# StefanHeng/Symbolic-Music-Generation

Hardware: AMD Instinct MI355X
Metric: train tokens/sec (TransfoXL seq2048 bf16), whole job (higher is better)
Workload: dtype bf16; 1 GPU; TransfoXL 12L/768d H12 dh64 F3072 T=2048 M=2048 V=1190 cutoffs=[] (SURVEY C3, mode R: fresh zero mems); per_gpu_batch=64, global_batch=64, seq_len=2048, mem_len=2048, parallelism=dp1

## Files before the change

### include/musicxl.h

```cpp
#ifndef MUSICXL_H
#define MUSICXL_H

#ifdef __cplusplus
extern "C" {
#endif

#define MXL_ABI_VERSION 2

int mxl_abi_version(void);
const char* mxl_error_string(int code);

#define MXL_GEMM_OUT_F32        0x01
#define MXL_GEMM_OUT_F32_ATOMIC 0x02
#define MXL_GEMM_BIAS           0x04
#define MXL_GEMM_RELU           0x08
#define MXL_GEMM_DROPOUT        0x10
#define MXL_GEMM_RELU_BWD       0x20
#define MXL_GEMM_ADD_AUX        0x40
int mxl_set_reserved_cus(int k);
int mxl_gemm_last_nt_kernel(void);

#define MXL_GEMM_SAVE_RELU_MASK 0x100
#define MXL_GEMM_RELU_BWD_BITS  0x200
size_t mxl_gemm_relu_mask_bytes(int M, int N);
// ... 46 lines not shown
int mxl_relattn_fwd_phantom(const void* q, const void* k, const void* v, const void* rd, const float* r_w_bias,
                            const float* r_r_bias, void* out, float* lse, void* oph, float* mph, int B, int T, int H,
                            int dh, int M, int Kc, long long q_bs, int q_rs, long long kv_bs, int kv_rs, int rd_rs,
                            long long o_bs, int o_rs, float scale, void* stream);
int mxl_relattn_bwd_sparse_dg_oph(const void* q, const void* k, const void* v, const void* rd, const float* r_w_bias,
                                  const float* r_r_bias, const void* out, const void* dout, const float* lse,
                                  float* delta, void* dq, void* dk, void* dv, void* dg, float* d_r_w_bias,
                                  const void* oph, const float* mph, int B, int T, int H, int dh, int M, int Kc,
                                  long long q_bs, int q_rs, long long kv_bs, int kv_rs, int rd_rs, long long o_bs, int o_rs,
                                  long long dq_bs, int dq_rs, long long dkv_bs, int dkv_rs, float scale, void* stream);
int mxl_relattn_drd_recompute(const void* dg, const void* qr, float* d_rd, int B, int T, int H, int dh, int M, long long qr_bs,
                              int qr_rs, int drd_ld, const void* rd, int rd_rs, float* d_r_r_bias, float* d_r_w_bias_fix,
                              const float* lse, const float* delta, float scale, int Kc, void* stream);

size_t mxl_relattn_bwd_fused_ws_bytes(int B, int T, int H, int dh, int M);
int mxl_relattn_bwd_fused(const void* q, const void* k, const void* v, const void* rd, const float* r_w_bias,
                          const float* r_r_bias, const void* out, const void* dout, const float* lse, float* delta,
                          void* dq, void* dk, void* dv, float* d_rd, int drd_ld, float* d_r_w_bias, float* d_r_r_bias,
                          const void* oph, const float* mph, void* ws, int B, int T, int H, int dh, int M, int Kc,
                          long long q_bs, int q_rs, long long kv_bs, int kv_rs, int rd_rs, long long o_bs, int o_rs,
                          long long dq_bs, int dq_rs, long long dkv_bs, int dkv_rs, float scale, int defer_finish, void* stream);
int mxl_relattn_dq_finish(const void* ws, const void* oph, const float* mph, const float* lse, const float* delta, void* dq,
                          float* d_r_r_bias, int B, int T, int H, int dh, int M, int Kc, long long o_bs, int o_rs, long long dq_bs,
                          int dq_rs, float scale, void* stream);
int mxl_relattn_fwd_phantom2(const void* q, const void* k, const void* v, const void* rd, const float* r_w_bias,
                             const float* r_r_bias, void* out, float* lse, void* oph, float* mph, int oph_all, void* ph_ws, int B,
                             int T, int H, int dh, int M, int Kc, long long q_bs, int q_rs, long long kv_bs, int kv_rs, int rd_rs,
                             long long o_bs, int o_rs, float scale, void* stream);
size_t mxl_relattn_drd_phantom_ws_bytes(int B, int T, int H);
int mxl_relattn_drd_phantom_prep(const void* q, long long q_bs, int q_rs, const float* r_r_bias, const float* lse, void* ws, int B, int T,
                                 int H, int dh, float scale, void* stream);
int mxl_relattn_drd_phantom(const void* ws, const float* delta, float* d_rd, int B, int T, int H, int dh, int M, int drd_ld,
                            const void* rd, int rd_rs, int Kc, void* stream);

int mxl_sinusoid_table(void* out, int M, int d, int clamp_len, float drop_p, unsigned long long seed, unsigned site,
                       void* stream);
int mxl_embed_fwd(const void* ids, const void* E, void* out, int N, int d, int V, float scale, float drop_p,
                  unsigned long long seed, unsigned site, void* stream);
int mxl_embed_bwd(const void* ids, const void* dout, const void* dout2, float* dE, int N, int d, int V, float scale,
                  float drop_p, unsigned long long seed, unsigned site, void* stream);
int mxl_dropout_bf16(const void* x, void* y, long long n, float drop_p, unsigned long long seed, unsigned site,
                     void* stream);
int mxl_ln_residual_fwd(const void* x, const void* res, const float* gamma, const float* beta, void* y, void* z,
                        float* mean, float* rstd, int N, int d, float eps, float drop_p, unsigned long long seed,
                        unsigned site, void* stream);
int mxl_ln_residual_bwd(const void* dy, const void* dy2, const void* z, const float* mean, const float* rstd,
                        const float* gamma, void* dres, void* dx, float* dgamma, float* dbeta, int N, int d,
                        float drop_p, unsigned long long seed, unsigned site, void* stream);
int mxl_ln_residual_bwd_colsum(const void* dy, const void* dy2, const void* z, const float* mean, const float* rstd,
                               const float* gamma, void* dres, void* dx, float* dgamma, float* dbeta, float* dxsum, int N,
                               int d, float drop_p, unsigned long long seed, unsigned site, void* stream);
int mxl_ln_residual_bwd_add(const void* dy, const void* dy2, const void* z, const float* mean, const float* rstd,
                            const float* gamma, const void* dadd, void* dres, float* dgamma, float* dbeta, int N, int d,
                            void* stream);
int mxl_ln_residual_bwd_add_drop(const void* dy, const void* dy2, const void* z, const float* mean, const float* rstd,
                                 const float* gamma, const void* dadd, void* dres, void* dx, float* dxsum, float* dgamma,
                                 float* dbeta, int N, int d, float drop_p, unsigned long long seed, unsigned site, void* stream);
int mxl_add_rowbias_bf16(const void* x, long long x_bs, int x_rs, const float* bias, void* out, int B, int T, int n,
                         void* stream);
int mxl_colsum_bf16(const void* X, float* out, int M, int N, int ld, void* stream);
int mxl_dropout_colsum_bf16(const void* X, void* Y, float* out, int M, int N, float drop_p, unsigned long long seed,
                            unsigned site, void* stream);
int mxl_center_columns_bf16(const void* X, void* Y, int M, int N, void* stream);
int mxl_mem_update(const void* mem, const void* hid, void* out, int B, int M, int T, int d, void* stream);

int mxl_label_guard(void* labels_row0, int T, long long eos, void* stream);
// ... 200 lines not shown
```

### symbolic_music_generation_amd/csrc/common.h

```cpp
#pragma once
#include <hip/hip_runtime.h>
#include <stdint.h>

#define MXL_OK 0
#define MXL_EINVAL (-1)
#define MXL_EUNSUPPORTED (-2)

#define MXL_CHECK_ARG(cond) do { if (!(cond)) return MXL_EINVAL; } while (0)
#define MXL_LAUNCH_CHECK() do { hipError_t e_ = hipGetLastError(); if (e_ != hipSuccess) return (int)e_; } while (0)

typedef uint16_t bf16_t;

using bf16x8 = __attribute__((ext_vector_type(8))) short;
using bf16x4 = __attribute__((ext_vector_type(4))) short;
using f32x4 = __attribute__((ext_vector_type(4))) float;
using f32x16 = __attribute__((ext_vector_type(16))) float;
using u32x4 = __attribute__((ext_vector_type(4))) uint32_t;
using u32x2 = __attribute__((ext_vector_type(2))) uint32_t;

__device__ __forceinline__ float bf2f(bf16_t x) { return __uint_as_float(((uint32_t)x) << 16); }

__device__ __forceinline__ bf16_t f2bf(float f) {
    __bf16 b = (__bf16)f;
    return __builtin_bit_cast(bf16_t, b);
}
__device__ __forceinline__ uint32_t pack2bf(float lo, float hi) {
    typedef __bf16 bf2_t __attribute__((ext_vector_type(2)));
    typedef float f2_t __attribute__((ext_vector_type(2)));
    f2_t v = {lo, hi};
    bf2_t r = __builtin_convertvector(v, bf2_t);
    return __builtin_bit_cast(uint32_t, r);
}

__device__ __forceinline__ void xcd_block(int& bx, int& by, int& bz) {
    const int gx = gridDim.x, gy = gridDim.y, groups = gridDim.y * gridDim.z;
#ifndef MXL_NO_XCD_REMAP
    const int L = blockIdx.x + gx * (blockIdx.y + gy * blockIdx.z);
    const int xcd = L & 7, idx = L >> 3;
    int grp;
    if ((groups & 7) == 0) {
        grp = (idx / gx) * 8 + xcd;
        bx = idx % gx;
    } else {
        const int n = gx * groups, q = n >> 3, r = n & 7;
        const int id = (xcd < r ? xcd * (q + 1) : r * (q + 1) + (xcd - r) * q) + idx;
        grp = id / gx;
        bx = id - grp * gx;
    }
    by = grp % gy; bz = grp / gy;
#else
    bx = blockIdx.x; by = blockIdx.y; bz = blockIdx.z;
#endif
}

__device__ __forceinline__ int lane_id() { return threadIdx.x & 63; }

__device__ __forceinline__ float wave_sum(float v) {
#pragma unroll
    for (int o = 32; o > 0; o >>= 1) v += __shfl_xor(v, o, 64);
    return v;
}
__device__ __forceinline__ float wave_max(float v) {
#pragma unroll
    for (int o = 32; o > 0; o >>= 1) v = fmaxf(v, __shfl_xor(v, o, 64));
    return v;
}

__device__ __forceinline__ uint32_t mxl_hash32(uint32_t x) {
    x ^= x >> 16; x *= 0x7feb352dU; x ^= x >> 15; x *= 0x846ca68bU; x ^= x >> 16;
    return x;
}
__device__ __forceinline__ bool dropout_keep(uint64_t seed, uint32_t site, uint64_t idx, uint32_t thresh) {
    const uint32_t mix = mxl_hash32((uint32_t)seed ^ (site * 0x9E3779B9U)) + (uint32_t)(seed >> 32);
    const uint32_t h = mxl_hash32(((uint32_t)idx * 0x9E3779B1U) ^ ((uint32_t)(idx >> 32) * 0x85EBCA77U) ^ mix);
    return h >= thresh;
}
__device__ __forceinline__ bool dropout_keep32(uint64_t seed, uint32_t site, uint32_t idx, uint32_t thresh) {
    const uint32_t mix = mxl_hash32((uint32_t)seed ^ (site * 0x9E3779B9U)) + (uint32_t)(seed >> 32);
    return mxl_hash32((idx * 0x9E3779B1U) ^ mix) >= thresh;
}
static inline uint32_t dropout_thresh(float p) {
// ... 6 lines not shown
```

### symbolic_music_generation_amd/csrc/relattn_bwd_fused.hip

```cpp
#include <cstdlib>
#include <type_traits>
#include "common.h"
#include "musicxl_internal.h"

namespace {

typedef __attribute__((ext_vector_type(8))) __bf16 mfma_bf16x8;
typedef __attribute__((address_space(3))) bf16x4 lds_bf16x4;
typedef _Float16 f16x4 __attribute__((ext_vector_type(4)));
typedef float f32x4v __attribute__((ext_vector_type(4)));

#ifndef FUSED_PF
#define FUSED_PF 3
#endif
#ifndef FUSED_VF_RELOAD
#define FUSED_VF_RELOAD 0
#endif
#ifndef FUSED_PARK
#define FUSED_PARK 0
#endif
#ifndef FUSED_SB
#define FUSED_SB 1
#endif
#define UNIT_FENCE() do { if (FUSED_SB) __builtin_amdgcn_sched_barrier(0); } while (0)
// ... 33 lines not shown
#ifdef MXL_STAMP
__device__ unsigned long long g_fused_stamps[16];
#define STAMP_DECL unsigned long long st_last, st_acc[16] = {0ull, 0ull, 0ull, 0ull, 0ull, 0ull, 0ull, 0ull, 0ull, 0ull, 0ull, 0ull, 0ull, 0ull, 0ull, 0ull}; \
    { __builtin_amdgcn_sched_barrier(0); asm volatile("s_memtime %0\n\ts_waitcnt lgkmcnt(0)" : "=s"(st_last) :: "memory"); __builtin_amdgcn_sched_barrier(0); }
#define STAMP(i) { unsigned long long t_; __builtin_amdgcn_sched_barrier(0); asm volatile("s_memtime %0\n\ts_waitcnt lgkmcnt(0)" : "=s"(t_) :: "memory"); \
    __builtin_amdgcn_sched_barrier(0); st_acc[i] += t_ - st_last; st_last = t_; }
#define STAMP_FLUSH if ((threadIdx.x & 63) == 0) { for (int i_ = 0; i_ < 16; i_++) atomicAdd(&g_fused_stamps[i_], st_acc[i_]); }
#else
#define STAMP_DECL
#define STAMP(i)
#define STAMP_FLUSH
#endif

#ifndef MXL_SLAB_BF16
#define MXL_SLAB_BF16 1
#endif
#if MXL_SLAB_BF16
typedef bf16_t slab_t;
#else
typedef float slab_t;
#endif

struct FusedP {
    const bf16_t *q, *k, *v, *rd, *dout;
    const float *rwb, *rrb, *lse, *delta;
    bf16_t *dk, *dv;
    slab_t* slab;
    float* drd;
    float *d_rwb, *d_rrb;
    int B, T, H, M, Kc;
    long long q_bs, kv_bs, o_bs, dkv_bs, slab_stride;
    int q_rs, kv_rs, rd_rs, o_rs, dkv_rs, drd_ld;
    float scale, scale_log2e;
};

__device__ __forceinline__ int qswz(int row) { return (((row >> 1) & 1) << 2) | (((row >> 2) & 1) << 1) | ((row >> 3) & 1); }
__device__ __forceinline__ int qoff(int row, int ch) { return row * ROWB + ((ch ^ qswz(row)) << 4); }
__device__ __forceinline__ int qeoff(int row, int e) { return qoff(row, e >> 3) + ((e & 7) << 1); }
__device__ __forceinline__ int sswz(int row) { return (((row >> 3) & 1) << 2) | (((row >> 1) & 1) << 1) | ((row >> 2) & 1); }
__device__ __forceinline__ int soff(int row, int ch) { return row * ROWB + ((ch ^ sswz(row)) << 4); }

__device__ __forceinline__ void lds_barrier() {
    asm volatile("s_waitcnt lgkmcnt(0)" ::: "memory");
    __builtin_amdgcn_s_barrier();
    asm volatile("" ::: "memory");
}

__device__ __forceinline__ uint32_t lds_addr(const void* p) {
    return (uint32_t)(uintptr_t)(__attribute__((address_space(3))) const char*)(const char*)p;
}

__device__ __forceinline__ void gskew_wait() { asm volatile("s_waitcnt lgkmcnt(0)" ::: "memory"); }
__device__ __forceinline__ void gskew_read16(uint32_t base, uint32_t (&u)[16]) {
    static_assert(GP == 584, "offsets below are pat(j) * (GP + 2)");
    asm volatile(
        "ds_read_u16 %0, %16\n\t"               "ds_read_u16 %1, %16 offset:586\n\t"    "ds_read_u16 %2, %16 offset:1172\n\t"
        "ds_read_u16 %3, %16 offset:1758\n\t"   "ds_read_u16 %4, %16 offset:4688\n\t"   "ds_read_u16 %5, %16 offset:5274\n\t"
        "ds_read_u16 %6, %16 offset:5860\n\t"   "ds_read_u16 %7, %16 offset:6446\n\t"   "ds_read_u16 %8, %16 offset:9376\n\t"
        "ds_read_u16 %9, %16 offset:9962\n\t"   "ds_read_u16 %10, %16 offset:10548\n\t" "ds_read_u16 %11, %16 offset:11134\n\t"
        "ds_read_u16 %12, %16 offset:14064\n\t" "ds_read_u16 %13, %16 offset:14650\n\t" "ds_read_u16 %14, %16 offset:15236\n\t"
        "ds_read_u16 %15, %16 offset:15822"
        : "=&v"(u[0]), "=&v"(u[1]), "=&v"(u[2]), "=&v"(u[3]), "=&v"(u[4]), "=&v"(u[5]), "=&v"(u[6]), "=&v"(u[7]),
          "=&v"(u[8]), "=&v"(u[9]), "=&v"(u[10]), "=&v"(u[11]), "=&v"(u[12]), "=&v"(u[13]), "=&v"(u[14]), "=&v"(u[15])
        : "v"(base)
        : "memory");
}
// ... 41 lines not shown
    const bf16_t* dp = dout + (size_t)b * o_bs + (size_t)i * o_rs;
    const int chunks = H * 8;
    for (int c0 = 0; c0 < chunks; c0 += 64) {
        const int c = c0 + lane;
        float s = 0.f;
        if (c < chunks) {
            const bf16x8 a = *reinterpret_cast<const bf16x8*>(op + c * 8);
            const bf16x8 d = *reinterpret_cast<const bf16x8*>(dp + c * 8);
#pragma unroll
            for (int j = 0; j < 8; j++) s += bf2f((bf16_t)a[j]) * bf2f((bf16_t)d[j]);
        }
        s += __shfl_xor(s, 1, 64); s += __shfl_xor(s, 2, 64); s += __shfl_xor(s, 4, 64);
        if (c < chunks && (lane & 7) == 0) delta[((size_t)b * H + (c >> 3)) * T + i] = s;
    }
}

__global__ __launch_bounds__(512, 1) void relattn_bwd_fused_kernel(FusedP p) {
    constexpr int NT = 512;
    extern __shared__ __attribute__((aligned(16))) char smem[];
    char* sK = smem;
    char* sR = sK + K_BYTES;
    char* sQ = sR + RING_BYTES;
    char* sG = sQ + 2 * QSET;
    char* sX = sG + G_BYTES;
    char* sY = sX + X_BYTES;
    float* sBias = reinterpret_cast<float*>(sY + Y_BYTES);
    float* sPark = sBias + BIAS_BYTES / 4;

    STAMP_DECL
    const int tid = threadIdx.x;
    const int w = __builtin_amdgcn_readfirstlane(tid >> 6);
    const int l = tid & 63, r = l & 31, hh = l >> 5;
    int bx_, h, b;
    xcd_block(bx_, h, b);
    const int T = p.T, M = p.M;
    const int p0 = T - p.Kc;
    const int P0 = p0 + KBLK * bx_;
    const int Pw = P0 + 32 * w;
    const int kloc0 = 32 * w + r;
    const int MB = M >> 5;

    const bf16_t* qbase = p.q + (size_t)b * p.q_bs + (size_t)h * 64;
    const bf16_t* dobase = p.dout + (size_t)b * p.o_bs + (size_t)h * 64;
    const bf16_t* rbase = p.rd + (size_t)h * 64;
    const bf16_t* kbase = p.k + (size_t)b * p.kv_bs + (size_t)h * 64;
    const bf16_t* vbase = p.v + (size_t)b * p.kv_bs + (size_t)h * 64;

    const int gq = l >> 4, q4 = (l & 15) >> 2, pp = l & 3;
    int rowq = qoff(r, hh);
    int rows = r * ROWB + ((hh ^ sswz(r)) << 4);
    int tkb = qeoff(4 * hh + q4, 16 * (gq & 1) + 4 * pp);
    const uint32_t gRb = lds_addr(sG) + 4 * hh * (GP + 2) + (256 - kloc0) * 2;
    const uint32_t yWb = lds_addr(sY) + 4 * hh * (YP + 2) + (256 - kloc0) * 2;
    const int xf = (kloc0 >> 1) & 7;
    int xw = kloc0 * 64 + ((((hh ^ (xf & 1)) | (xf & 6))) << 3);
    int yt0 = (4 * (l >> 4) + ((l & 15) >> 2)) * YP + (16 * (w & 1) + 4 * pp) * 2;
    int qb0 = qeoff(4 * (l >> 4) + ((l & 15) >> 2), 16 * (w >> 1) + 4 * pp);
    const int eq = w >> 1, ih0 = w & 1;
    const int g16 = l >> 4, q16 = (l & 15) >> 2;
    int xa0 = ((8 * g16 + q16) * 64 + ((pp ^ ((4 * g16 + (q16 >> 1)) & 7)) << 3)) ^ (ih0 << 5);
    int xa1 = ((8 * g16 + q16 + 4) * 64 + ((pp ^ ((4 * g16 + 2 + (q16 >> 1)) & 7)) << 3)) ^ (ih0 << 5);
    const int kch = 2 * eq + (pp >> 1);
    const int ksw = ((g16 & 1) << 2) | (((q16 >> 1) & 1) << 1);
    int ka0 = (8 * g16 + q16) * ROWB + ((kch ^ ksw) << 4) + ((pp & 1) << 3);
    int ka1 = (8 * g16 + q16 + 4) * ROWB + ((kch ^ (ksw | 1)) << 4) + ((pp & 1) << 3);
    int yq0 = (16 * ih0 + (l & 15)) * YP + 16 * g16;
    int krow = kloc0 * ROWB + ((hh ^ sswz(kloc0)) << 4);
// ... 649 lines not shown
    MXL_CHECK_ARG(q && k && v && rd && r_w_bias && r_r_bias && out && dout && lse && delta && dq && dk && dv && d_rd && d_r_w_bias &&
                  d_r_r_bias && ws);
    if (dh != 64) return MXL_EUNSUPPORTED;
    MXL_CHECK_ARG(B > 0 && T > 0 && H > 0 && M > 0 && Kc >= T && Kc <= M + T && drd_ld >= H * 64);
    if ((T % 32) != 0 || (M % 32) != 0 || (Kc % 32) != 0) return MXL_EUNSUPPORTED;
    MXL_CHECK_ARG(Kc == M + T || (oph && mph));
    MXL_CHECK_ARG((q_rs % 8) == 0 && (kv_rs % 8) == 0 && (rd_rs % 8) == 0 && (o_rs % 8) == 0 && (dq_rs % 8) == 0 && (dkv_rs % 4) == 0);
    MXL_CHECK_ARG((q_bs % 8) == 0 && (kv_bs % 8) == 0 && (o_bs % 8) == 0 && (dq_bs % 8) == 0 && (dkv_bs % 4) == 0);
    MXL_CHECK_ARG(((uintptr_t)q % 16) == 0 && ((uintptr_t)k % 16) == 0 && ((uintptr_t)v % 16) == 0 && ((uintptr_t)rd % 16) == 0 &&
                  ((uintptr_t)out % 16) == 0 && ((uintptr_t)dout % 16) == 0 && ((uintptr_t)dq % 16) == 0 && ((uintptr_t)ws % 16) == 0 &&
                  (oph == nullptr || ((uintptr_t)oph % 16) == 0));
    hipStream_t s = (hipStream_t)stream;
    static bool attr_set = false;
    if (!attr_set) {
        hipError_t e = hipFuncSetAttribute(reinterpret_cast<const void*>(&relattn_bwd_fused_kernel), hipFuncAttributeMaxDynamicSharedMemorySize, SMEM);
        if (e != hipSuccess) return (int)e;
        attr_set = true;
    }
    const bool delta_ready = (defer_finish & 2) != 0;
    defer_finish &= 1;
    if (!delta_ready) {
        mxl_kt::Scope kt(MXL_KT_RELATTN_DELTA, s);
        hipLaunchKernelGGL(fused_delta_kernel, dim3((B * T + 3) / 4), dim3(256), 0, s, (const bf16_t*)out, (const bf16_t*)dout, delta, B, T,
                           H, o_bs, o_rs);
    }
    FusedP p;
    p.q = (const bf16_t*)q; p.k = (const bf16_t*)k; p.v = (const bf16_t*)v; p.rd = (const bf16_t*)rd; p.dout = (const bf16_t*)dout;
    p.rwb = r_w_bias; p.rrb = r_r_bias; p.lse = lse; p.delta = delta;
    p.dk = (bf16_t*)dk; p.dv = (bf16_t*)dv; p.slab = (slab_t*)ws; p.drd = d_rd; p.d_rwb = d_r_w_bias; p.d_rrb = d_r_r_bias;
    p.B = B; p.T = T; p.H = H; p.M = M; p.Kc = Kc;
    p.q_bs = q_bs; p.kv_bs = kv_bs; p.o_bs = o_bs; p.dkv_bs = dkv_bs; p.slab_stride = (long long)B * T * H * 64;
    p.q_rs = q_rs; p.kv_rs = kv_rs; p.rd_rs = rd_rs; p.o_rs = o_rs; p.dkv_rs = dkv_rs; p.drd_ld = drd_ld;
    p.scale = scale; p.scale_log2e = scale * LOG2E;
    {
        mxl_kt::Scope kt(MXL_KT_RELATTN_FUSED, s);
        hipLaunchKernelGGL(relattn_bwd_fused_kernel, dim3((Kc + KBLK - 1) / KBLK, H, B), dim3(512), SMEM, s, p);
    }
    MXL_LAUNCH_CHECK();
    if (defer_finish) return MXL_OK;
    return mxl_relattn_dq_finish(ws, oph, mph, lse, delta, dq, d_r_r_bias, B, T, H, dh, M, Kc, o_bs, o_rs, dq_bs, dq_rs, scale, stream);
}

extern "C" int mxl_relattn_dq_finish(const void* ws, const void* oph, const float* mph, const float* lse, const float* delta, void* dq,
                                     float* d_r_r_bias, int B, int T, int H, int dh, int M, int Kc, long long o_bs, int o_rs,
                                     long long dq_bs, int dq_rs, float scale, void* stream) {
    MXL_CHECK_ARG(ws && lse && delta && dq && B > 0 && T > 0 && H > 0 && M > 0 && Kc >= T && Kc <= M + T);
    if (dh != 64 || (T % 32) != 0 || (M % 32) != 0 || (Kc % 32) != 0) return MXL_EUNSUPPORTED;
    MXL_CHECK_ARG(Kc == M + T || (oph && mph));
    MXL_CHECK_ARG((o_rs % 8) == 0 && (o_bs % 8) == 0 && (dq_rs % 8) == 0 && (dq_bs % 8) == 0 && ((uintptr_t)dq % 16) == 0 &&
                  ((uintptr_t)ws % 16) == 0 && (oph == nullptr || ((uintptr_t)oph % 16) == 0));
    hipStream_t s = (hipStream_t)stream;
    FinP f;
    f.slab = (const slab_t*)ws; f.oph = (Kc < M + T) ? (const bf16_t*)oph : nullptr; f.mph = mph; f.lse = lse; f.delta = delta;
    f.dq = (bf16_t*)dq; f.d_rrb = d_r_r_bias;
    f.B = B; f.T = T; f.H = H; f.M = M; f.Kc = Kc;
    f.slab_stride = (long long)B * T * H * 64; f.o_bs = o_bs; f.dq_bs = dq_bs; f.o_rs = o_rs; f.dq_rs = dq_rs; f.scale = scale;
    {
        mxl_kt::Scope kt(MXL_KT_RELATTN_DQFIN, s);
        const long long rgs = (long long)B * (T / FIN_ROWS);
        const int nch = H * 8, cw = nch < 256 ? nch : 256, busy = (256 / cw) * cw, nthr = (busy + 63) / 64 * 64;
        static const int per_cu = getenv("MXL_DQFIN_WG_PER_CU") ? atoi(getenv("MXL_DQFIN_WG_PER_CU")) : 2048 / nthr;
        const long long want = 256ll * per_cu;
        hipLaunchKernelGGL(relattn_dq_finish_kernel, dim3((unsigned)(rgs < want ? rgs : want)), dim3(nthr), 0, s, f);
    }
    MXL_LAUNCH_CHECK();
    return MXL_OK;
}
```

### symbolic_music_generation_amd/csrc/relattn_drd_phantom.hip

```cpp
#include "common.h"
#include "musicxl_internal.h"

namespace {

typedef __attribute__((ext_vector_type(8))) __bf16 mfma_bf16x8;
typedef __attribute__((address_space(3))) void* lptr_t;
constexpr float LOG2E = 1.4426950408889634f;

__device__ __forceinline__ float mul1(float a, float b) {
    float r;
    asm("v_mul_f32 %0, %1, %2" : "=v"(r) : "v"(a), "v"(b));
    return r;
}
__device__ __forceinline__ f32x16 mfma32(bf16x8 a, bf16x8 b, f32x16 c) {
    return __builtin_amdgcn_mfma_f32_32x32x16_bf16(__builtin_bit_cast(mfma_bf16x8, a), __builtin_bit_cast(mfma_bf16x8, b), c, 0, 0, 0);
}
typedef unsigned long long u64x2 __attribute__((ext_vector_type(2)));
__device__ __forceinline__ void tr_read8(uint32_t a0, uint32_t a1, bf16x8 (&fb)[2][2]) {
    u64x2 v00, v01, v10, v11;
    asm volatile(
        "ds_read_b64_tr_b16 %0, %8\n\tds_read_b64_tr_b16 %1, %9 offset:1024\n\t"
        "ds_read_b64_tr_b16 %2, %8 offset:2048\n\tds_read_b64_tr_b16 %3, %9 offset:3072\n\t"
        "ds_read_b64_tr_b16 %4, %10\n\tds_read_b64_tr_b16 %5, %11 offset:1024\n\t"
        "ds_read_b64_tr_b16 %6, %10 offset:2048\n\tds_read_b64_tr_b16 %7, %11 offset:3072\n\t"
// ... 22 lines not shown
    for (int j = 0; j < 8; j++) o[j] = (bf2f((bf16_t)v[j]) + rrb[c * 8 + j]) * scale_log2e;
    const u32x4 w = {pack2bf(o[0], o[1]), pack2bf(o[2], o[3]), pack2bf(o[4], o[5]), pack2bf(o[6], o[7])};
    const int r = t & 31;
    char* dst = rec + (((size_t)b * H + (c >> 3)) * (T >> 5) + (t >> 5)) * PH_REC + r * 128 + (((c & 7) ^ ph_swz(r)) << 4);
    *reinterpret_cast<u32x4*>(dst) = w;
}
__global__ void phantom_prep_sc_kernel(const float* lse, char* rec, long long n, int T) {
    const long long i = (long long)blockIdx.x * blockDim.x + threadIdx.x;
    if (i >= n) return;
    const long long bh = i / T;
    const int t = (int)(i % T);
    reinterpret_cast<float*>(rec + (bh * (T >> 5) + (t >> 5)) * PH_REC + 4096)[t & 31] = -lse[i] * LOG2E;
}

#ifdef MXL_STAMP
__device__ unsigned long long g_ph_stamps[16];
#define STAMP_DECL unsigned long long st_last, st_acc[16] = {0ull, 0ull, 0ull, 0ull, 0ull, 0ull, 0ull, 0ull, 0ull, 0ull, 0ull, 0ull, 0ull, 0ull, 0ull, 0ull}; \
    { __builtin_amdgcn_sched_barrier(0); asm volatile("s_memtime %0\n\ts_waitcnt lgkmcnt(0)" : "=s"(st_last) :: "memory"); __builtin_amdgcn_sched_barrier(0); }
#define STAMP(i) { unsigned long long t_; __builtin_amdgcn_sched_barrier(0); asm volatile("s_memtime %0\n\ts_waitcnt lgkmcnt(0)" : "=s"(t_) :: "memory"); \
    __builtin_amdgcn_sched_barrier(0); st_acc[i] += t_ - st_last; st_last = t_; }
#define STAMP_FLUSH if ((threadIdx.x & 63) == 0) { for (int i_ = 0; i_ < 16; i_++) atomicAdd(&g_ph_stamps[i_], st_acc[i_]); }
#else
#define STAMP_DECL
#define STAMP(i)
#define STAMP_FLUSH
#endif

struct PhP {
    const char* rec; const float* delta; const bf16_t* rd; float* drd;
    int B, T, H, M, bgroup;
    int rd_rs, drd_ld;
    float scale; int pz;
    int mk[32];
};
constexpr int PH_STAGE = PH_REC + 256;
#ifndef PH_NST_
#define PH_NST_ 16
#endif
constexpr int PH_NST = PH_NST_, PH_PA = PH_NST_ - 4;
constexpr int PH_SMEM = PH_STAGE * PH_NST;


__global__ __launch_bounds__(256, 2) void relattn_drd_phantom_kernel(PhP p) {
    extern __shared__ __attribute__((aligned(1024))) char smem[];
    const int wid = __builtin_amdgcn_readfirstlane(threadIdx.x >> 6), l = threadIdx.x & 63, r = l & 31, hh = l >> 5;
    int bx_, h, bz_;
    xcd_block(bx_, h, bz_);
    STAMP_DECL
    bx_ = gridDim.x - 1 - bx_;
    const int d0 = bx_ * 256;
    const int mk = p.mk[bx_ & 31];
    if (bz_ & (mk - 1)) return;
    const int b0 = bz_ * p.bgroup;
    const int nb = min(p.bgroup * mk, p.B - b0);
    const int spb = p.T >> 5;
    const int tph = (d0 + p.pz) >> 5;
    const int nph = max(0, min(spb, tph + 8));
    const int SA = nb * nph;
    if (SA <= 0) return;
    const int tb0 = tph + 2 * wid;

    bf16x8 rdf[2][4];
#pragma unroll
    for (int nt = 0; nt < 2; nt++)
#pragma unroll
        for (int ks = 0; ks < 4; ks++) {
            const int dd = d0 + 64 * wid + 32 * nt + r;
            const bf16x8 zz = {0, 0, 0, 0, 0, 0, 0, 0};
            rdf[nt][ks] = dd < p.M ? *reinterpret_cast<const bf16x8*>(p.rd + (size_t)dd * p.rd_rs + h * 64 + 16 * ks + 8 * hh) : zz;
        }
    const int A0 = r * 128 + ((hh ^ ph_swz(r)) << 4);
    const int q4 = (l & 15) >> 2, pp = l & 3, cg_ = (l >> 4) & 1;
    const int B0 = (4 * hh + q4) * 128 + ((((2 * cg_ + (pp >> 1)) ^ (4 * ((q4 >> 1) & 1) + 2 * hh))) << 4) + ((pp & 1) << 3);
    const int sv0 = 4096 + 16 * hh;

    const int rec_b = p.H * spb * PH_REC;
    const __amdgpu_buffer_rsrc_t rs_dl = __builtin_amdgcn_make_buffer_rsrc((void*)p.delta, 0, p.B * p.H * p.T * 4, 0x00020000);
    int ib = b0, it = 0, ig = 0;
    auto issue = [&]() {
        char* st = smem + (ig & (PH_NST - 1)) * PH_STAGE;
        const __amdgpu_buffer_rsrc_t rs = __builtin_amdgcn_make_buffer_rsrc((void*)(p.rec + (size_t)ib * rec_b), 0, -1, 0x00020000);
        const int so = (h * spb + it) * PH_REC;
        __builtin_amdgcn_raw_ptr_buffer_load_lds(rs, (lptr_t)(st + wid * 1024), 16, wid * 1024 + l * 16, so, 0, 0);
        if (wid == 0) __builtin_amdgcn_raw_ptr_buffer_load_lds(rs, (lptr_t)(st + 4096), 4, 4096 + l * 4, so, 0, 0);
        if (wid == 1) __builtin_amdgcn_raw_ptr_buffer_load_lds(rs_dl, (lptr_t)(st + PH_REC), 4, l * 4, (((ib * p.H + h) * spb + it) * 32) * 4, 0, 0);
        ig++;
        if (++it == nph) { it = 0; ib++; }
    };
    auto wait_ring = [&]() {
        if (wid < 2) asm volatile("s_waitcnt vmcnt(%0)" :: "n"(2 * (PH_PA - 2)) : "memory");
        else asm volatile("s_waitcnt vmcnt(%0)" :: "n"(PH_PA - 2) : "memory");
    };

    f32x16 acc[2][2];
#pragma unroll
    for (int nt = 0; nt < 2; nt++)
#pragma unroll
        for (int et = 0; et < 2; et++)
#pragma unroll
            for (int t = 0; t < 16; t++) acc[nt][et][t] = 0.f;

    auto ld16 = [&](const char* a) {
        f32x16 c;
#pragma unroll
        for (int g4 = 0; g4 < 4; g4++) {
            const f32x4 v = *reinterpret_cast<const f32x4*>(a + 32 * g4);
#pragma unroll
            for (int j = 0; j < 4; j++) c[4 * g4 + j] = v[j];
        }
        return c;
    };
    auto ld_qa = [&](const char* st, bf16x8 (&qa)[4]) {
#pragma unroll
        for (int ks = 0; ks < 4; ks++) qa[ks] = *reinterpret_cast<const bf16x8*>(st + (A0 ^ (ks << 5)));
    };
    const uint32_t lds0 = (uint32_t)(uintptr_t)(__attribute__((address_space(3))) char*)smem;
    auto gprod = [&](const bf16x8 (&qa)[4], int nt, f32x16 c) {
#pragma unroll
// ... 3 lines not shown
    auto pexp = [&](const f32x16& c, const f32x16& nd, bool diag, bf16x8 (&pa)[2]) {
        float pv[16];
        if (!diag) {
#pragma unroll
            for (int t = 0; t < 16; t++) pv[t] = mul1(__builtin_amdgcn_exp2f(c[t]), nd[t]);
        } else {
            const int tl = r - 4 * hh;
#pragma unroll
            for (int t = 0; t < 16; t++) {
                const bool valid = tl >= (t & 3) + 8 * (t >> 2) + 1;
                pv[t] = mul1(__builtin_amdgcn_exp2f(valid ? c[t] : -1.0e30f), nd[t]);
            }
        }
#pragma unroll
        for (int s = 0; s < 2; s++) {
            const u32x4 w = {pack2bf(pv[8 * s], pv[8 * s + 1]), pack2bf(pv[8 * s + 2], pv[8 * s + 3]),
                             pack2bf(pv[8 * s + 4], pv[8 * s + 5]), pack2bf(pv[8 * s + 6], pv[8 * s + 7])};
            pa[s] = __builtin_bit_cast(bf16x8, w);
        }
    };
    auto contract = [&](const bf16x8 (&pa)[2], const bf16x8 (&fb)[2][2], int nt) {
#pragma unroll
        for (int s = 0; s < 2; s++)
#pragma unroll
            for (int et = 0; et < 2; et++) acc[nt][et] = mfma32(pa[s], fb[et][s], acc[nt][et]);
    };

    for (int g = 0; g < min(PH_PA, SA); g++) issue();
    if (SA >= PH_PA) wait_ring();
    else asm volatile("s_waitcnt vmcnt(0)" ::: "memory");
    __builtin_amdgcn_s_barrier();
    bf16x8 qa0[4], qa1[4];
    f32x16 cg0, cg1;
    int tc = 0;
    ld_qa(smem, qa0);
    cg0 = ld16(smem + sv0);
    if (tc <= tb0) cg0 = gprod(qa0, 0, cg0);
    STAMP(15)
    auto step = [&](int g, bf16x8 (&qa)[4], f32x16& cgA, bf16x8 (&qaN)[4], f32x16& cgN, const bool odd) {
        STAMP(0)
        const char* st = smem + (g & (PH_NST - 1)) * PH_STAGE;
        const char* stN = smem + ((g + 1) & (PH_NST - 1)) * PH_STAGE;
        const bool more = g + 1 < SA;
        const int tcN = (tc + 1 == nph) ? 0 : tc + 1;
        const bool uA = tc <= tb0, uB = tc <= tb0 + 1;
        f32x16 cgB = ld16(st + sv0);
        const f32x16 nd = ld16(st + sv0 + 256);
        if (uB) cgB = gprod(qa, 1, cgB);
        STAMP(1)
        bf16x8 fb[2][2];
        {
            const uint32_t sb = lds0 + (g & (PH_NST - 1)) * PH_STAGE + B0;
            tr_read8(sb, sb ^ 64u, fb);
        }
        STAMP(2)
        if (odd) {
            if (g + PH_PA < SA) wait_ring();
            else asm volatile("s_waitcnt vmcnt(0)" ::: "memory");
            asm volatile("s_waitcnt lgkmcnt(0)" ::: "memory");
            __builtin_amdgcn_s_barrier();
        }
        STAMP(3)
        bf16x8 paA[2];
        if (uA) pexp(cgA, nd, tc == tb0, paA);
        STAMP(4)
        if (more) { ld_qa(stN, qaN); cgN = ld16(stN + sv0); }
        STAMP(5)
        if (uA) contract(paA, fb, 0);
        STAMP(6)
        if (more && tcN <= tb0) cgN = gprod(qaN, 0, cgN);
        STAMP(7)
        if (uB) {
            bf16x8 pa[2];
            pexp(cgB, nd, tc == tb0 + 1, pa);
            STAMP(8)
            contract(pa, fb, 1);
        }
        STAMP(9)
        tc = tcN;
    };
#pragma unroll 1
    for (int g = 0; g < SA; g += 2) {
        if (g + PH_PA < SA) issue();
        if (g + PH_PA + 1 < SA) issue();
        step(g, qa0, cg0, qa1, cg1, false);
        if (g + 1 < SA) step(g + 1, qa1, cg1, qa0, cg0, true);
    }

    const float nsc = -1.f / LOG2E;
#pragma unroll
    for (int nt = 0; nt < 2; nt++)
#pragma unroll
        for (int t = 0; t < 16; t++) {
            const int dd = d0 + 64 * wid + 32 * nt + (t & 3) + 8 * (t >> 2) + 4 * hh;
            float* dst = p.drd + (size_t)dd * p.drd_ld + h * 64 + r;
            if (dd < p.M) {
#pragma unroll
                for (int et = 0; et < 2; et++) atomicAdd(dst + 32 * et, acc[nt][et][t] * nsc);
            }
        }
    STAMP(14)
    STAMP_FLUSH
}

}

#ifdef MXL_STAMP
extern "C" int mxl_debug_phantom_occupancy() {
    int n = -1;
    hipFuncSetAttribute(reinterpret_cast<const void*>(&relattn_drd_phantom_kernel), hipFuncAttributeMaxDynamicSharedMemorySize, PH_SMEM);
    hipError_t e = hipOccupancyMaxActiveBlocksPerMultiprocessor(&n, relattn_drd_phantom_kernel, 256, PH_SMEM);
    return e == hipSuccess ? n : -(int)e;
}
extern "C" int mxl_debug_phantom_stamps(unsigned long long* host_out16) {
    hipError_t e = hipMemcpyFromSymbol(host_out16, HIP_SYMBOL(g_ph_stamps), sizeof(unsigned long long) * 16);
    if (e != hipSuccess) return (int)e;
    unsigned long long z[16] = {0};
    e = hipMemcpyToSymbol(HIP_SYMBOL(g_ph_stamps), z, sizeof(z));
    return (int)e;
}
#endif

extern "C" size_t mxl_relattn_drd_phantom_ws_bytes(int B, int T, int H) {
    if (B <= 0 || T <= 0 || H <= 0 || (T % 32) != 0) return 0;
    return (size_t)B * H * (T / 32) * PH_REC;
}

extern "C" int mxl_relattn_drd_phantom_prep(const void* q, long long q_bs, int q_rs, const float* r_r_bias, const float* lse, void* ws,
                                            int B, int T, int H, int dh, float scale, void* stream) {
    MXL_CHECK_ARG(q && r_r_bias && lse && ws && B > 0 && T > 0 && H > 0);
    if (dh != 64 || (T % 32) != 0) return MXL_EUNSUPPORTED;
    MXL_CHECK_ARG((q_rs % 8) == 0 && (q_bs % 8) == 0 && ((uintptr_t)q % 16) == 0 && ((uintptr_t)ws % 16) == 0);
    const long long tot = (long long)B * T * (H * 8), nsc = (long long)B * H * T;
    {
        mxl_kt::Scope kt(MXL_KT_ROWBIAS, (hipStream_t)stream);
        hipLaunchKernelGGL(phantom_prep_kernel, dim3((unsigned)((tot + 255) / 256)), dim3(256), 0, (hipStream_t)stream, (const bf16_t*)q,
                           q_bs, q_rs, r_r_bias, (char*)ws, B, T, H, scale * LOG2E);
        hipLaunchKernelGGL(phantom_prep_sc_kernel, dim3((unsigned)((nsc + 255) / 256)), dim3(256), 0, (hipStream_t)stream, lse,
                           (char*)ws, nsc, T);
    }
    MXL_LAUNCH_CHECK();
    return MXL_OK;
}

extern "C" int mxl_relattn_drd_phantom(const void* ws, const float* delta, float* d_rd, int B, int T, int H, int dh, int M, int drd_ld,
                                       const void* rd, int rd_rs, int Kc, void* stream) {
    MXL_CHECK_ARG(ws && delta && d_rd && rd && B > 0 && T > 0 && H > 0 && M > 0 && Kc >= T && Kc <= M + T);
    if (dh != 64 || (T % 32) != 0 || (M % 32) != 0 || (M + 255) / 256 > 32) return MXL_EUNSUPPORTED;
    MXL_CHECK_ARG(((T - Kc) % 64) == 0);
    MXL_CHECK_ARG((rd_rs % 8) == 0 && drd_ld >= H * 64 && ((uintptr_t)ws % 16) == 0 && ((uintptr_t)rd % 16) == 0);
    MXL_CHECK_ARG((long long)H * (T / 32) * PH_REC < (1ll << 31) && (long long)B * H * T * 4 < (1ll << 31));
    if (Kc >= M + T) return MXL_OK;
    static bool attr_set = false;
    if (!attr_set) {
        hipError_t e = hipFuncSetAttribute(reinterpret_cast<const void*>(&relattn_drd_phantom_kernel),
                                           hipFuncAttributeMaxDynamicSharedMemorySize, PH_SMEM);
        if (e != hipSuccess) return (int)e;
        attr_set = true;
    }
    PhP p;
    p.rec = (const char*)ws; p.delta = delta; p.rd = (const bf16_t*)rd; p.drd = d_rd;
    p.B = B; p.T = T; p.H = H; p.M = M; p.rd_rs = rd_rs; p.drd_ld = drd_ld;
    p.scale = 0.f; p.pz = T - Kc;
    const int nk = (M + 255) / 256, spb = T / 32;
    int nph[32], ref = 0;
    for (int k = 0; k < nk; k++) {
        const int v = (256 * k + p.pz) / 32 + 8;
        nph[k] = (256 * k + p.pz < -256) ? 0 : (v < 0 ? 0 : (v > spb ? spb : v));
        if (nph[k] > ref) ref = nph[k];
    }
    if (ref == 0) return MXL_OK;
    const int tiles = nk * H;
    static const int fac = getenv("MXL_DRD_PH_FACTOR") ? atoi(getenv("MXL_DRD_PH_FACTOR")) : 6;
    int groups = (fac * 512 + tiles - 1) / tiles;
    if (groups < 1) groups = 1;
    if (groups > B) groups = B;
    p.bgroup = (B + groups - 1) / groups;
    groups = (B + p.bgroup - 1) / p.bgroup;
    static const int balance = getenv("MXL_DRD_PH_BALANCE") ? atoi(getenv("MXL_DRD_PH_BALANCE")) : 0;
    for (int k = 0; k < 32; k++) {
        int m = 1;
        if (balance && k < nk && nph[k] > 0) while (2 * m * nph[k] <= ref && 2 * m <= groups) m *= 2;
        p.mk[k] = m;
    }
    {
        mxl_kt::Scope kt(MXL_KT_RELATTN_DRD, (hipStream_t)stream);
        hipLaunchKernelGGL(relattn_drd_phantom_kernel, dim3(nk, H, groups), dim3(256), PH_SMEM, (hipStream_t)stream, p);
    }
    MXL_LAUNCH_CHECK();
    return MXL_OK;
}
```

Baseline: 860,400 tokens/s.

## Split drd phantom kernel into unmasked fast range and generic launch; reorder fused bwd grid

The relative-attention d_rd phantom kernel now splits each column's time-block range into a fully-unmasked prefix and the remainder. The prefix runs a FAST template instantiation that skips the per-step causal masking checks, and the remainder uses the generic kernel, each launch with its own grid-group sizing. Separately, the fused backward kernel's block order is changed so that the long-running column tiles are scheduled first, with XCD-aware ordering applied within each class, to reduce tail imbalance. The cost is an extra kernel launch, more host-side planning and several new env knobs.

Result: faster. 879,200 tokens/s, median of 6 (+2.2%).

```diff
diff --git a/include/musicxl.h b/include/musicxl.h
--- a/include/musicxl.h
+++ b/include/musicxl.h
@@ -102,6 +102,8 @@
                                  int H, int dh, float scale, void* stream);
 int mxl_relattn_drd_phantom(const void* ws, const float* delta, float* d_rd, int B, int T, int H, int dh, int M, int drd_ld,
                             const void* rd, int rd_rs, int Kc, void* stream);
+int mxl_debug_phantom_split(int B, int T, int M, int Kc, long long* out4);
+int mxl_debug_phantom_occupancy(int fast);
 
 int mxl_sinusoid_table(void* out, int M, int d, int clamp_len, float drop_p, unsigned long long seed, unsigned site,
                        void* stream);
diff --git a/symbolic_music_generation_amd/csrc/common.h b/symbolic_music_generation_amd/csrc/common.h
--- a/symbolic_music_generation_amd/csrc/common.h
+++ b/symbolic_music_generation_amd/csrc/common.h
@@ -1,6 +1,7 @@
 #pragma once
 #include <hip/hip_runtime.h>
 #include <stdint.h>
+#include "grid_order.h"
 
 #define MXL_OK 0
 #define MXL_EINVAL (-1)
@@ -36,17 +37,8 @@
     const int gx = gridDim.x, gy = gridDim.y, groups = gridDim.y * gridDim.z;
 #ifndef MXL_NO_XCD_REMAP
     const int L = blockIdx.x + gx * (blockIdx.y + gy * blockIdx.z);
-    const int xcd = L & 7, idx = L >> 3;
     int grp;
-    if ((groups & 7) == 0) {
-        grp = (idx / gx) * 8 + xcd;
-        bx = idx % gx;
-    } else {
-        const int n = gx * groups, q = n >> 3, r = n & 7;
-        const int id = (xcd < r ? xcd * (q + 1) : r * (q + 1) + (xcd - r) * q) + idx;
-        grp = id / gx;
-        bx = id - grp * gx;
-    }
+    xcd_order(L, gx, groups, bx, grp);
     by = grp % gy; bz = grp / gy;
 #else
     bx = blockIdx.x; by = blockIdx.y; bz = blockIdx.z;
diff --git a/symbolic_music_generation_amd/csrc/grid_order.h b/symbolic_music_generation_amd/csrc/grid_order.h
--- /dev/null
+++ b/symbolic_music_generation_amd/csrc/grid_order.h
@@ -0,0 +1,45 @@
+#pragma once
+
+#if defined(__HIPCC__) || defined(__CUDACC__)
+#define MXL_HD __host__ __device__ __forceinline__
+#else
+#define MXL_HD inline
+#endif
+
+MXL_HD void xcd_order(int L, int gx, int groups, int& bx, int& grp) {
+    const int xcd = L & 7, idx = L >> 3;
+    if ((groups & 7) == 0) {
+        grp = (idx / gx) * 8 + xcd;
+        bx = idx % gx;
+    } else {
+        const int n = gx * groups, q = n >> 3, r = n & 7;
+        const int id = (xcd < r ? xcd * (q + 1) : r * (q + 1) + (xcd - r) * q) + idx;
+        grp = id / gx;
+        bx = id - grp * gx;
+    }
+}
+
+MXL_HD void fused_order(int L, int gx, int gy, int gz, int gx_long, int* bx, int* h, int* b) {
+    const int groups = gy * gz, n_long = gx_long * groups;
+    int x, grp;
+    if (L < n_long) {
+        xcd_order(L, gx_long, groups, x, grp);
+    } else {
+        xcd_order(L - n_long, gx - gx_long, groups, x, grp);
+        x += gx_long;
+    }
+    *bx = x; *h = grp % gy; *b = grp / gy;
+}
+
+MXL_HD int fused_gx_long(int T, int M, int Kc, int gx) {
+    int longest = 0, last_long = -1;
+    for (int pass = 0; pass < 2; pass++)
+        for (int x = 0; x < gx; x++) {
+            const int P0 = T - Kc + 256 * x;
+            const int lo = P0 > 0 ? P0 : 0, hi = P0 + 255 + M - 1 < T - 1 ? P0 + 255 + M - 1 : T - 1;
+            const int len = hi >= lo ? (hi >> 5) - (lo >> 5) + 1 : 0;
+            if (pass == 0) { if (len > longest) longest = len; }
+            else if (4 * len > longest) last_long = x;
+        }
+    return last_long + 1 > 0 ? last_long + 1 : gx;
+}
diff --git a/symbolic_music_generation_amd/csrc/relattn_bwd_fused.hip b/symbolic_music_generation_amd/csrc/relattn_bwd_fused.hip
--- a/symbolic_music_generation_amd/csrc/relattn_bwd_fused.hip
+++ b/symbolic_music_generation_amd/csrc/relattn_bwd_fused.hip
@@ -89,6 +89,7 @@
     long long q_bs, kv_bs, o_bs, dkv_bs, slab_stride;
     int q_rs, kv_rs, rd_rs, o_rs, dkv_rs, drd_ld;
     float scale, scale_log2e;
+    int gx_long;
 };
 
 __device__ __forceinline__ int qswz(int row) { return (((row >> 1) & 1) << 2) | (((row >> 2) & 1) << 1) | ((row >> 3) & 1); }
@@ -196,7 +197,7 @@
     const int w = __builtin_amdgcn_readfirstlane(tid >> 6);
     const int l = tid & 63, r = l & 31, hh = l >> 5;
     int bx_, h, b;
-    xcd_block(bx_, h, b);
+    fused_order(blockIdx.x + gridDim.x * (blockIdx.y + gridDim.y * blockIdx.z), gridDim.x, gridDim.y, gridDim.z, p.gx_long, &bx_, &h, &b);
     const int T = p.T, M = p.M;
     const int p0 = T - p.Kc;
     const int P0 = p0 + KBLK * bx_;
@@ -912,9 +913,13 @@
     p.q_bs = q_bs; p.kv_bs = kv_bs; p.o_bs = o_bs; p.dkv_bs = dkv_bs; p.slab_stride = (long long)B * T * H * 64;
     p.q_rs = q_rs; p.kv_rs = kv_rs; p.rd_rs = rd_rs; p.o_rs = o_rs; p.dkv_rs = dkv_rs; p.drd_ld = drd_ld;
     p.scale = scale; p.scale_log2e = scale * LOG2E;
+    const int gx = (Kc + KBLK - 1) / KBLK;
+    const char *ord_env = getenv("MXL_FUSED_ORDER"), *gxl_env = getenv("MXL_FUSED_GX_LONG");
+    p.gx_long = (ord_env && atoi(ord_env) == 0) ? gx : fused_gx_long(T, M, Kc, gx);
+    if (gxl_env && !(ord_env && atoi(ord_env) == 0)) p.gx_long = atoi(gxl_env) < 0 ? 0 : (atoi(gxl_env) > gx ? gx : atoi(gxl_env));
     {
         mxl_kt::Scope kt(MXL_KT_RELATTN_FUSED, s);
-        hipLaunchKernelGGL(relattn_bwd_fused_kernel, dim3((Kc + KBLK - 1) / KBLK, H, B), dim3(512), SMEM, s, p);
+        hipLaunchKernelGGL(relattn_bwd_fused_kernel, dim3(gx, H, B), dim3(512), SMEM, s, p);
     }
     MXL_LAUNCH_CHECK();
     if (defer_finish) return MXL_OK;
diff --git a/symbolic_music_generation_amd/csrc/relattn_drd_phantom.hip b/symbolic_music_generation_amd/csrc/relattn_drd_phantom.hip
--- a/symbolic_music_generation_amd/csrc/relattn_drd_phantom.hip
+++ b/symbolic_music_generation_amd/csrc/relattn_drd_phantom.hip
@@ -78,6 +78,7 @@
     int rd_rs, drd_ld;
     float scale; int pz;
     int mk[32];
+    int t0[32], t1[32];
 };
 constexpr int PH_STAGE = PH_REC + 256;
 #ifndef PH_NST_
@@ -87,6 +88,7 @@
 constexpr int PH_SMEM = PH_STAGE * PH_NST;
 
 
+template <bool FAST>
 __global__ __launch_bounds__(256, 2) void relattn_drd_phantom_kernel(PhP p) {
     extern __shared__ __attribute__((aligned(1024))) char smem[];
     const int wid = __builtin_amdgcn_readfirstlane(threadIdx.x >> 6), l = threadIdx.x & 63, r = l & 31, hh = l >> 5;
@@ -101,9 +103,9 @@
     const int nb = min(p.bgroup * mk, p.B - b0);
     const int spb = p.T >> 5;
     const int tph = (d0 + p.pz) >> 5;
-    const int nph = max(0, min(spb, tph + 8));
+    const int tlo = p.t0[bx_ & 31], nph = p.t1[bx_ & 31] - tlo;
     const int SA = nb * nph;
-    if (SA <= 0) return;
+    if (nph <= 0 || SA <= 0) return;
     const int tb0 = tph + 2 * wid;
 
     bf16x8 rdf[2][4];
@@ -126,10 +128,10 @@
     auto issue = [&]() {
         char* st = smem + (ig & (PH_NST - 1)) * PH_STAGE;
         const __amdgpu_buffer_rsrc_t rs = __builtin_amdgcn_make_buffer_rsrc((void*)(p.rec + (size_t)ib * rec_b), 0, -1, 0x00020000);
-        const int so = (h * spb + it) * PH_REC;
+        const int so = (h * spb + tlo + it) * PH_REC;
         __builtin_amdgcn_raw_ptr_buffer_load_lds(rs, (lptr_t)(st + wid * 1024), 16, wid * 1024 + l * 16, so, 0, 0);
         if (wid == 0) __builtin_amdgcn_raw_ptr_buffer_load_lds(rs, (lptr_t)(st + 4096), 4, 4096 + l * 4, so, 0, 0);
-        if (wid == 1) __builtin_amdgcn_raw_ptr_buffer_load_lds(rs_dl, (lptr_t)(st + PH_REC), 4, l * 4, (((ib * p.H + h) * spb + it) * 32) * 4, 0, 0);
+        if (wid == 1) __builtin_amdgcn_raw_ptr_buffer_load_lds(rs_dl, (lptr_t)(st + PH_REC), 4, l * 4, (((ib * p.H + h) * spb + tlo + it) * 32) * 4, 0, 0);
         ig++;
         if (++it == nph) { it = 0; ib++; }
     };
@@ -199,18 +201,18 @@
     __builtin_amdgcn_s_barrier();
     bf16x8 qa0[4], qa1[4];
     f32x16 cg0, cg1;
-    int tc = 0;
+    int tc = tlo;
     ld_qa(smem, qa0);
     cg0 = ld16(smem + sv0);
-    if (tc <= tb0) cg0 = gprod(qa0, 0, cg0);
+    if (FAST || tc <= tb0) cg0 = gprod(qa0, 0, cg0);
     STAMP(15)
     auto step = [&](int g, bf16x8 (&qa)[4], f32x16& cgA, bf16x8 (&qaN)[4], f32x16& cgN, const bool odd) {
         STAMP(0)
         const char* st = smem + (g & (PH_NST - 1)) * PH_STAGE;
         const char* stN = smem + ((g + 1) & (PH_NST - 1)) * PH_STAGE;
         const bool more = g + 1 < SA;
-        const int tcN = (tc + 1 == nph) ? 0 : tc + 1;
-        const bool uA = tc <= tb0, uB = tc <= tb0 + 1;
+        const int tcN = (tc + 1 == tlo + nph) ? tlo : tc + 1;
+        const bool uA = FAST || tc <= tb0, uB = FAST || tc <= tb0 + 1;
         f32x16 cgB = ld16(st + sv0);
         const f32x16 nd = ld16(st + sv0 + 256);
         if (uB) cgB = gprod(qa, 1, cgB);
@@ -229,22 +231,22 @@
         }
         STAMP(3)
         bf16x8 paA[2];
-        if (uA) pexp(cgA, nd, tc == tb0, paA);
+        if (uA) pexp(cgA, nd, !FAST && tc == tb0, paA);
         STAMP(4)
         if (more) { ld_qa(stN, qaN); cgN = ld16(stN + sv0); }
         STAMP(5)
         if (uA) contract(paA, fb, 0);
         STAMP(6)
-        if (more && tcN <= tb0) cgN = gprod(qaN, 0, cgN);
+        if (more && (FAST || tcN <= tb0)) cgN = gprod(qaN, 0, cgN);
         STAMP(7)
         if (uB) {
             bf16x8 pa[2];
-            pexp(cgB, nd, tc == tb0 + 1, pa);
+            pexp(cgB, nd, !FAST && tc == tb0 + 1, pa);
             STAMP(8)
             contract(pa, fb, 1);
         }
         STAMP(9)
-        tc = tcN;
+        if (!FAST) tc = tcN;
     };
 #pragma unroll 1
     for (int g = 0; g < SA; g += 2) {
@@ -272,13 +274,50 @@
 
 }
 
+struct PhPlan { int nk, t0[2][32], t1[2][32], cols[2], longest[2]; long long steps[2]; };
+static PhPlan ph_plan(int B, int T, int M, int pz, bool split) {
+    PhPlan pl;
+    pl.nk = (M + 255) / 256;
+    const int spb = T / 32;
+    for (int f = 0; f < 2; f++) { pl.cols[f] = pl.longest[f] = 0; pl.steps[f] = 0; }
+    for (int k = 0; k < 32; k++) {
+        int nph = 0, tph = 0;
+        if (k < pl.nk && 256 * k + pz >= -256) {
+            tph = (256 * k + pz) / 32;
+            nph = tph + 8 < 0 ? 0 : (tph + 8 > spb ? spb : tph + 8);
+        }
+        const int cut = (!split || 256 * k + 256 > M) ? 0 : (tph < 0 ? 0 : (tph > nph ? nph : tph));
+        pl.t0[1][k] = 0; pl.t1[1][k] = cut;
+        pl.t0[0][k] = cut; pl.t1[0][k] = nph;
+        for (int f = 0; f < 2; f++) {
+            const int n = pl.t1[f][k] - pl.t0[f][k];
+            if (n > 0) { pl.cols[f]++; pl.steps[f] += (long long)B * n; if (n > pl.longest[f]) pl.longest[f] = n; }
+        }
+    }
+    return pl;
+}
+static int ph_split_mode() {
+    const char* e = getenv("MXL_DRD_PH_SPLIT");
+    return !e ? 1 : (atoi(e) == 0 ? 0 : (atoi(e) == 2 ? 2 : 1));
+}
+
+extern "C" int mxl_debug_phantom_occupancy(int fast) {
+    int n = -1;
+    const void* fn = fast ? reinterpret_cast<const void*>(&relattn_drd_phantom_kernel<true>) : reinterpret_cast<const void*>(&relattn_drd_phantom_kernel<false>);
+    hipError_t e = hipFuncSetAttribute(fn, hipFuncAttributeMaxDynamicSharedMemorySize, PH_SMEM);
+    if (e != hipSuccess) return -(int)e;
+    e = fast ? hipOccupancyMaxActiveBlocksPerMultiprocessor(&n, relattn_drd_phantom_kernel<true>, 256, PH_SMEM)
+             : hipOccupancyMaxActiveBlocksPerMultiprocessor(&n, relattn_drd_phantom_kernel<false>, 256, PH_SMEM);
+    return e == hipSuccess ? n : -(int)e;
+}
+extern "C" int mxl_debug_phantom_split(int B, int T, int M, int Kc, long long* out4) {
+    MXL_CHECK_ARG(out4 && B > 0 && T > 0 && M > 0 && Kc >= T && Kc <= M + T && (T % 32) == 0 && (M % 32) == 0 && (M + 255) / 256 <= 32);
+    const int split = ph_split_mode();
+    const PhPlan pl = ph_plan(B, T, M, T - Kc, split != 0), all = ph_plan(B, T, M, T - Kc, false);
+    out4[0] = pl.steps[0]; out4[1] = pl.steps[1]; out4[2] = all.steps[0]; out4[3] = split;
+    return MXL_OK;
+}
 #ifdef MXL_STAMP
-extern "C" int mxl_debug_phantom_occupancy() {
-    int n = -1;
-    hipFuncSetAttribute(reinterpret_cast<const void*>(&relattn_drd_phantom_kernel), hipFuncAttributeMaxDynamicSharedMemorySize, PH_SMEM);
-    hipError_t e = hipOccupancyMaxActiveBlocksPerMultiprocessor(&n, relattn_drd_phantom_kernel, 256, PH_SMEM);
-    return e == hipSuccess ? n : -(int)e;
-}
 extern "C" int mxl_debug_phantom_stamps(unsigned long long* host_out16) {
     hipError_t e = hipMemcpyFromSymbol(host_out16, HIP_SYMBOL(g_ph_stamps), sizeof(unsigned long long) * 16);
     if (e != hipSuccess) return (int)e;
@@ -320,8 +359,11 @@
     if (Kc >= M + T) return MXL_OK;
     static bool attr_set = false;
     if (!attr_set) {
-        hipError_t e = hipFuncSetAttribute(reinterpret_cast<const void*>(&relattn_drd_phantom_kernel),
+        hipError_t e = hipFuncSetAttribute(reinterpret_cast<const void*>(&relattn_drd_phantom_kernel<false>),
                                            hipFuncAttributeMaxDynamicSharedMemorySize, PH_SMEM);
+        if (e == hipSuccess)
+            e = hipFuncSetAttribute(reinterpret_cast<const void*>(&relattn_drd_phantom_kernel<true>),
+                                    hipFuncAttributeMaxDynamicSharedMemorySize, PH_SMEM);
         if (e != hipSuccess) return (int)e;
         attr_set = true;
     }
@@ -329,30 +371,31 @@
     p.rec = (const char*)ws; p.delta = delta; p.rd = (const bf16_t*)rd; p.drd = d_rd;
     p.B = B; p.T = T; p.H = H; p.M = M; p.rd_rs = rd_rs; p.drd_ld = drd_ld;
     p.scale = 0.f; p.pz = T - Kc;
-    const int nk = (M + 255) / 256, spb = T / 32;
-    int nph[32], ref = 0;
-    for (int k = 0; k < nk; k++) {
-        const int v = (256 * k + p.pz) / 32 + 8;
-        nph[k] = (256 * k + p.pz < -256) ? 0 : (v < 0 ? 0 : (v > spb ? spb : v));
-        if (nph[k] > ref) ref = nph[k];
-    }
-    if (ref == 0) return MXL_OK;
-    const int tiles = nk * H;
+    const int split = ph_split_mode();
+    const PhPlan pl = ph_plan(B, T, M, p.pz, split != 0);
+    if (pl.steps[0] + pl.steps[1] == 0) return MXL_OK;
     static const int fac = getenv("MXL_DRD_PH_FACTOR") ? atoi(getenv("MXL_DRD_PH_FACTOR")) : 6;
-    int groups = (fac * 512 + tiles - 1) / tiles;
-    if (groups < 1) groups = 1;
-    if (groups > B) groups = B;
-    p.bgroup = (B + groups - 1) / groups;
-    groups = (B + p.bgroup - 1) / p.bgroup;
+    static const int fac_gen = getenv("MXL_DRD_PH_FACTOR_GEN") ? atoi(getenv("MXL_DRD_PH_FACTOR_GEN")) : 3;
     static const int balance = getenv("MXL_DRD_PH_BALANCE") ? atoi(getenv("MXL_DRD_PH_BALANCE")) : 0;
-    for (int k = 0; k < 32; k++) {
-        int m = 1;
-        if (balance && k < nk && nph[k] > 0) while (2 * m * nph[k] <= ref && 2 * m <= groups) m *= 2;
-        p.mk[k] = m;
-    }
     {
         mxl_kt::Scope kt(MXL_KT_RELATTN_DRD, (hipStream_t)stream);
-        hipLaunchKernelGGL(relattn_drd_phantom_kernel, dim3(nk, H, groups), dim3(256), PH_SMEM, (hipStream_t)stream, p);
+        for (int f = 1; f >= 0; f--) {
+            if (pl.steps[f] == 0) continue;
+            const int tiles = (pl.steps[1] > 0 ? pl.cols[f] : pl.nk) * H;
+            int groups = ((f == 0 && pl.steps[1] > 0 ? fac_gen : fac) * 512 + tiles - 1) / tiles;
+            if (groups < 1) groups = 1;
+            if (groups > B) groups = B;
+            p.bgroup = (B + groups - 1) / groups;
+            groups = (B + p.bgroup - 1) / p.bgroup;
+            for (int k = 0; k < 32; k++) {
+                const int n = pl.t1[f][k] - pl.t0[f][k];
+                int m = 1;
+                if (balance && n > 0) while (2 * m * n <= pl.longest[f] && 2 * m <= groups) m *= 2;
+                p.mk[k] = m; p.t0[k] = pl.t0[f][k]; p.t1[k] = pl.t1[f][k];
+            }
+            if (f && split != 2) hipLaunchKernelGGL(relattn_drd_phantom_kernel<true>, dim3(pl.nk, H, groups), dim3(256), PH_SMEM, (hipStream_t)stream, p);
+            else hipLaunchKernelGGL(relattn_drd_phantom_kernel<false>, dim3(pl.nk, H, groups), dim3(256), PH_SMEM, (hipStream_t)stream, p);
+        }
     }
     MXL_LAUNCH_CHECK();
     return MXL_OK;
```
